# DUBSON0/iterative-closest-point-avmi

Measured on AMD Instinct MI355X. Metric: icp_iterations_per_sec, higher is better.
Workload: dtype f64

## Files before the change

### iterative-closest-point-avmi_amd/csrc/icp2.hip

```cpp
#include <cstdlib>

#include "linalg.hpp"
#include "prep_common.hpp"
#include "sweep.hpp"

namespace icpmi {


struct Icp2Args {
    const double* pts;
    const int32_t* off;
    const int32_t* cnt;
    const int32_t* pair_src;
    const int32_t* pair_tgt;
    const double* init;
    double* results;
    const double2* g_sxy;
    const double2* g_snrm;
    const int32_t* g_sorig;
    const float* g_skey;
    const int32_t* g_dir;
    int lds_points;
    double error_threshold;
    double max_corr_dist;
    int max_iterations;
    int method;
    int has_init;
    int n_lo, m_lo;
    int skip_over;
    int it_begin, it_limit;
    int resume;
    double2* st_xy;
    int32_t* st_pos;
    int32_t* list;
    int32_t* list_count;
    int st_stride;
    int32_t* wide_list;
    int32_t* wide_count;
    int32_t* far_list;
    int32_t* far_count;
    double far_d2;
    IcpGate gate;
};
constexpr int ICP2_FAR_THREADS = 1024, ICP2_FAR_SMAX = 2, ICP2_FAR_POINTS = 2048;
constexpr int ICP2_ST_PARKED = 100;

__device__ __forceinline__ double swap_add(double a, double b, bool rows16) {
    const long long ab = __double_as_longlong(a), bb = __double_as_longlong(b);
    const unsigned alo = (unsigned)ab, ahi = (unsigned)(ab >> 32), blo = (unsigned)bb, bhi = (unsigned)(bb >> 32);
    unsigned xl, xh, yl, yh;
    if (rows16) {
        const auto r0 = __builtin_amdgcn_permlane16_swap(alo, blo, false, false);
        const auto r1 = __builtin_amdgcn_permlane16_swap(ahi, bhi, false, false);
        xl = r0[0]; yl = r0[1]; xh = r1[0]; yh = r1[1];
    } else {
        const auto r0 = __builtin_amdgcn_permlane32_swap(alo, blo, false, false);
        const auto r1 = __builtin_amdgcn_permlane32_swap(ahi, bhi, false, false);
        xl = r0[0]; yl = r0[1]; xh = r1[0]; yh = r1[1];
    }
    return __longlong_as_double(((long long)xh << 32) | xl) + __longlong_as_double(((long long)yh << 32) | yl);
}

constexpr int RED_MAXW = 16;
template <int NV>
constexpr int red_doubles() { return (NV + 3) / 4 * 4 * RED_MAXW; }

template <int NV>
__device__ __forceinline__ void wave_totals(double* scratch, const double (&v)[NV]) {
    constexpr int NP = (NV + 3) / 4 * 4;
    const int w = wave_id(), l = lane_id();
    double h[NP / 2];
#pragma unroll
    for (int j = 0; j < NP / 2; ++j)
        h[j] = swap_add(2 * j < NV ? v[2 * j] : 0.0, 2 * j + 1 < NV ? v[2 * j + 1] : 0.0, false);
#pragma unroll
    for (int k = 0; k < NP / 4; ++k) {
        const double q = row_sum(swap_add(h[2 * k], h[2 * k + 1], true));
        const int row = l >> 4;
        const int idx = 4 * k + ((row & 1) << 1) + (row >> 1);
        if ((l & 15) == 0 && idx < NV) scratch[idx * RED_MAXW + w] = q;
    }
}

template <int NV>
__device__ __forceinline__ void combine_totals(const double* scratch, int n_waves, double (&v)[NV]) {
    const int l = lane_id();
    double s = 0.0;
    if (l < NV)
        for (int w = 0; w < n_waves; ++w) s += scratch[l * RED_MAXW + w];
#pragma unroll
    for (int i = 0; i < NV; ++i) v[i] = readlane_f64(s, i);
}

constexpr int CTRL_R = 0, CTRL_T = 4, CTRL_STOP = 6, CTRL_MP = 8, CTRL_MQ = 10;
constexpr int CTRL_RT = 12, CTRL_TT = 16, CTRL_ERR = 18, CTRL_PREV = 19, CTRL_DELTA = 20, CTRL_ITERS = 21, CTRL_STATUS = 22,
              CTRL_DOUBLES = 24;

#ifndef ICP2_STAGE1_ITERS
#define ICP2_STAGE1_ITERS 12
#endif
#ifndef ICP2_PK_MIN
#define ICP2_PK_MIN 16
#endif
#ifndef ICP2_PLAIN_ITERS
#define ICP2_PLAIN_ITERS 2
#endif
#ifndef ICP2_CENTRED_ITERS
#define ICP2_CENTRED_ITERS 2
#endif
#ifndef ICP2_PLAIN_CENTRED
#define ICP2_PLAIN_CENTRED ICP2_PLAIN_ITERS
#endif
__device__ __forceinline__ double wave_uniform(double v) {
    const long long b = __double_as_longlong(v);
    const unsigned lo = __builtin_amdgcn_readfirstlane((unsigned)b), hi = __builtin_amdgcn_readfirstlane((unsigned)(b >> 32));
    return __longlong_as_double((long long)(((unsigned long long)hi << 32) | lo));
}
__device__ __forceinline__ float wave_uniform(float v) {
    return __int_as_float(__builtin_amdgcn_readfirstlane(__float_as_int(v)));
}

constexpr int FIN_GO = 0, FIN_STOP = 1, FIN_FAR = 2;
__device__ __forceinline__ int finish_step(double* ctrl, int it, double err_sum, double inliers, int N, bool has_corr,
                                           int need, double error_threshold, bool writer, double far_err) {
    bool stop = false, far = false;
    if (it > 0) {
        const double err = err_sum / (double)N, delta = fabs(ctrl[CTRL_PREV] - err);
        stop = delta < error_threshold;
        far = it == 1 && err > far_err;
        if (writer) {
            ctrl[CTRL_ERR] = err; ctrl[CTRL_DELTA] = delta; ctrl[CTRL_PREV] = err; ctrl[CTRL_ITERS] = (double)it;
            if (stop) ctrl[CTRL_STATUS] = (double)ICPMI_ST_CONVERGED;
        }
    }
    if (!stop && has_corr && inliers < (double)need) {
        stop = true;
        if (writer) { ctrl[CTRL_STATUS] = (double)ICPMI_ST_FEW_INLIERS; ctrl[CTRL_ITERS] = (double)it; }
    }
    return stop ? FIN_STOP : (far ? FIN_FAR : FIN_GO);
}

__device__ __forceinline__ int gate_stop(double* ctrl, const int32_t* hint, int gate_seen, int gate_index, bool writer, int fin) {
    if (fin == FIN_STOP || !hint || __builtin_amdgcn_readfirstlane(gate_seen) >= gate_index) return fin;
    if (writer) ctrl[CTRL_STATUS] = (double)ICPMI_ST_SKIPPED;
    return FIN_STOP;
}

__device__ __forceinline__ void accumulate_step(double* ctrl, const double (&r)[4], const double (&t)[2]) {
    const double rt0 = ctrl[CTRL_RT], rt1 = ctrl[CTRL_RT + 1], rt2 = ctrl[CTRL_RT + 2], rt3 = ctrl[CTRL_RT + 3];
    const double tt0 = ctrl[CTRL_TT], tt1 = ctrl[CTRL_TT + 1];
    ctrl[CTRL_RT] = r[0] * rt0 + r[1] * rt2; ctrl[CTRL_RT + 1] = r[0] * rt1 + r[1] * rt3;
    ctrl[CTRL_RT + 2] = r[2] * rt0 + r[3] * rt2; ctrl[CTRL_RT + 3] = r[2] * rt1 + r[3] * rt3;
    ctrl[CTRL_TT] = (tt0 * r[0] + tt1 * r[1]) + t[0]; ctrl[CTRL_TT + 1] = (tt0 * r[2] + tt1 * r[3]) + t[1];
}

union FarSlot {
    struct { double x, y; int seed, pad; } in;
    struct { double s1, s3; int p1, p2; } out;
};
static_assert(sizeof(FarSlot) == 24, "24 B per row");

template <int THREADS, int ICP2_SMAX, bool TGT_LDS, bool FILT, bool RESUME, bool FAR = false>
__device__ __forceinline__ void icp2_pair(const Icp2Args& a, const int b) {
    extern __shared__ __attribute__((aligned(16))) unsigned char dyn[];
    __shared__ double redA[red_doubles<11>()];
    __shared__ double redB[red_doubles<4>()];
    __shared__ double ctrl[CTRL_DOUBLES];
    constexpr int NWAVES = THREADS / ICPMI_WAVE;

    const int tid = threadIdx.x;
    const bool lead = tid < ICPMI_WAVE;
    const int sc = a.pair_src[b], tc = a.pair_tgt[b];
    const int N = a.cnt ? a.cnt[sc] : a.off[sc + 1] - a.off[sc];
    const int M = a.cnt ? a.cnt[tc] : a.off[tc + 1] - a.off[tc];
    const double* src = a.pts + (size_t)a.off[sc] * 2;
    double* res = a.results + (size_t)b * ICPMI_RES_DOUBLES;
    const int dir = a.g_dir[tc];
    if (a.skip_over ? (N > THREADS * ICP2_SMAX || (TGT_LDS && M > a.lds_points)) : (a.n_lo >= 0 && N <= a.n_lo && M <= a.m_lo)) {
        if (a.skip_over && a.wide_list && threadIdx.x == 0) a.wide_list[atomicAdd(a.wide_count, 1)] = b;
        return;
    }
    const int gate_index = a.gate.base + b * a.gate.stride;
    if (RESUME && a.gate.hint) {
        __shared__ int gate_skip;
        if (tid == 0) {
            gate_skip = __hip_atomic_load(a.gate.hint, __ATOMIC_RELAXED, __HIP_MEMORY_SCOPE_AGENT) < gate_index;
            if (gate_skip) {
                res[ICPMI_RES_ITERS] += 1.0;
                res[ICPMI_RES_STATUS] = (double)ICPMI_ST_SKIPPED;
            }
        }
        __syncthreads();
        if (gate_skip) return;
    }
// ... 89 lines not shown
                    px[s] = sx; py[s] = sy;
                } else { px[s] = x; py[s] = y; }
            }
        }
        const bool has_corr = a.max_corr_dist >= 0.0;
        const double max_corr_sq = wave_uniform(a.max_corr_dist * a.max_corr_dist);
        const int need = max(3, N / 10);
        __syncthreads();
        if constexpr (FAR) {
            sweepf_build_tree(lds_sq, M, lds_tree, tree_leaves, tid, THREADS);
            __syncthreads();
        }
        const double2 c_lo = sxy[0], c_hi = sxy[M - 1];
        const double uabs = wave_uniform(fmax(fabs(proj(dir, c_lo.x, c_lo.y)), fabs(proj(dir, c_hi.x, c_hi.y))));
        if constexpr (FILT) {
            filt.rt = wave_uniform(__int_as_float(rt_bits) * 1.000001f);
            filt.ut = wave_uniform(fmaxf(fabsf(lds_sq[0].z), fabsf(lds_sq[M - 1].z)) * 1.000001f);
        }

        double e_part = 0.0;
        if (RESUME) {
#pragma unroll
            for (int s = 0; s < ICP2_SMAX; ++s) {
                if (!(s < S && s * THREADS + tid < N)) continue;
                const double2 q = sxy[pos[s]];
                const double ex = q.x - px[s], ey = q.y - py[s];
                double se = 0.0;
                se += ex * ex;
                se += ey * ey;
                e_part += se;
            }
        }
        bool stopped = false;
        const double far_err = !RESUME && a.max_iterations > 2 && N <= ICP2_FAR_THREADS * ICP2_FAR_SMAX && M <= ICP2_FAR_POINTS
                                   ? a.far_d2 : __builtin_inf();
        const int it_end = RESUME ? a.max_iterations : min(a.max_iterations, a.it_limit);
        for (int it = RESUME ? a.it_begin : 0; it < it_end; ++it) {
            int gate_seen = 0x7fffffff;
            if (a.gate.hint && tid == 0) gate_seen = __hip_atomic_load(a.gate.hint, __ATOMIC_RELAXED, __HIP_MEMORY_SCOPE_AGENT);
            bool srch[ICP2_SMAX];
#pragma unroll
            for (int s = 0; s < ICP2_SMAX; ++s) {
                const bool valid = s < S && s * THREADS + tid < N;
                bool within;
                if constexpr (FAR) {
                    within = false;
                    if (valid && budget[s] > 0.0f) {
                        const int pa = pos[s], pb = pos2[s] >= 0 ? pos2[s] : pos[s];
                        const double2 c = sxy[pa], e = sxy[pb];
                        const double dx = px[s] - c.x, dy = py[s] - c.y;
                        const double ex = px[s] - e.x, ey = py[s] - e.y;
                        double q2 = 0.0, w2 = 0.0;
                        q2 += dx * dx;
                        q2 += dy * dy;
                        w2 += ex * ex;
                        w2 += ey * ey;
                        const double g = (double)budget[s] - (fabs(px[s] - (double)ax[s]) + fabs(py[s] - (double)ay[s])) * 1.000000001;
                        within = g > 0.0 && fmin(q2, w2) * 1.000000000001 < g * g * 0.999999999999;
                    }
                } else {
                    within = valid && (fabs(px[s] - (double)ax[s]) + fabs(py[s] - (double)ay[s])) * 1.000000001 < (double)budget[s];
                }
                srch[s] = valid && !within;
                if (within) {
                    const int pa = pos[s], pb = pos2[s] >= 0 ? pos2[s] : pos[s];
                    const double2 c = sxy[pa], e = sxy[pb];
                    const double dx = px[s] - c.x, dy = py[s] - c.y;
                    const double ex = px[s] - e.x, ey = py[s] - e.y;
                    double q2 = 0.0, w2 = 0.0;
                    q2 += dx * dx;
                    q2 += dy * dy;
                    w2 += ex * ex;
                    w2 += ey * ey;
                    bool second_wins = w2 < q2;
                    if (w2 == q2 && pb != pa) {
                        if constexpr (FILT) second_wins = sweepf_row(lds_sq[pb]) < sweepf_row(lds_sq[pa]);
                        else second_wins = sorig[pb] < sorig[pa];
                    }
                    pos[s] = second_wins ? pb : pa;
                    pos2[s] = pos2[s] >= 0 ? (second_wins ? pa : pb) : -1;
                }
            }
            if (!RESUME && it < ICP2_PLAIN_ITERS) {
#pragma unroll
                for (int s = 0; s < ICP2_SMAX; ++s)
                    if (srch[s]) {
                        double d2s;
                        if constexpr (FILT) {
                            if (__popcll(__ballot(true)) >= ICP2_PK_MIN)
                                pos[s] = sweepf_nn_pk(lds_sq, sxy, filt, M, dir, uabs, px[s], py[s], pos[s], it < ICP2_PLAIN_CENTRED);
                            else pos[s] = sweepf_nn(lds_sq, sxy, filt, M, dir, uabs, px[s], py[s], pos[s], it < ICP2_PLAIN_CENTRED, d2s);
                        }
                        else pos[s] = sweep_nn(sxy, sorig, M, dir, uabs, px[s], py[s], pos[s], it < ICP2_PLAIN_CENTRED, d2s);
                    }
            } else {
                const bool centred = !RESUME && it < ICP2_CENTRED_ITERS;
                int slot[ICP2_SMAX];
                if constexpr (FAR) {
                    int nq = 0;
#pragma unroll
                    for (int s = 0; s < ICP2_SMAX; ++s) {
                        const unsigned long long bal = __ballot(srch[s]);
                        slot[s] = nq + (int)__builtin_amdgcn_mbcnt_hi((unsigned)(bal >> 32), __builtin_amdgcn_mbcnt_lo((unsigned)bal, 0u));
                        nq += __popcll(bal);
                        if (srch[s]) {
                            FarSlot e;
                            e.in.x = px[s]; e.in.y = py[s]; e.in.seed = pos[s]; e.in.pad = 0;
                            far_q[slot[s]] = e;
                        }
                    }
                    __builtin_amdgcn_fence(__ATOMIC_ACQ_REL, "wavefront");
                    __builtin_amdgcn_wave_barrier();
                    for (int j = tid & (ICPMI_WAVE - 1); j < nq; j += ICPMI_WAVE) {
                        const FarSlot e = far_q[j];
                        const Top2 r = sweepf_top2_far(lds_sq, sxy, lds_tree, tree_leaves, filt, M, dir, uabs, e.in.x, e.in.y, e.in.seed);
                        FarSlot o;
                        o.out.s1 = r.s1; o.out.s3 = r.s3; o.out.p1 = r.p1; o.out.p2 = r.p2;
                        far_q[j] = o;
                    }
                    __builtin_amdgcn_fence(__ATOMIC_ACQ_REL, "wavefront");
                    __builtin_amdgcn_wave_barrier();
                }
#pragma unroll
                for (int s = 0; s < ICP2_SMAX; ++s)
                    if (srch[s]) {
                        Top2 t2;
                        if constexpr (FAR) {
                            const FarSlot o = far_q[slot[s]];
                            t2.p1 = o.out.p1; t2.p2 = o.out.p2; t2.s1 = o.out.s1; t2.s2 = o.out.s1; t2.s3 = o.out.s3;
                        }
                        else if constexpr (FILT) {
                            if (__popcll(__ballot(true)) >= ICP2_PK_MIN)
                                t2 = sweepf_top2_pk(lds_sq, sxy, filt, M, dir, uabs, px[s], py[s], pos[s], centred);
                            else t2 = sweepf_top2(lds_sq, sxy, filt, M, dir, uabs, px[s], py[s], pos[s], centred);
                        }
                        else t2 = sweep_top2(sxy, sorig, M, dir, uabs, px[s], py[s], pos[s], centred);
                        pos[s] = t2.p1; pos2[s] = t2.p2;
                        float bf;
                        if constexpr (FAR) {
                            const double d1 = sqrt(t2.s1), d3 = sqrt(t2.s3);
                            bf = (float)(d3 - 1e-13 * (d3 + d1) - 1.3e-7 * (fabs(px[s]) + fabs(py[s])));
                        } else {
                            const float r3 = __builtin_amdgcn_sqrtf((float)t2.s3) * 0.9999997f;
                            const float r1 = __builtin_amdgcn_sqrtf((float)t2.s1) * 1.0000003f + 1e-30f;
                            bf = (r3 - r1) * 0.4999999f - 1.3e-7f * (fabsf((float)px[s]) + fabsf((float)py[s]));
                        }
                        bf = bf - fabsf(bf) * 1e-6f;
                        budget[s] = t2.s3 < __builtin_inf() ? bf : __builtin_inff();
                        ax[s] = (float)px[s]; ay[s] = (float)py[s];
                    }
            }
            bool in[ICP2_SMAX];
#pragma unroll
            for (int s = 0; s < ICP2_SMAX; ++s) in[s] = s < S && s * THREADS + tid < N;
            if (use_p2l) {
                double acc[11] = {0, 0, 0, 0, 0, 0, 0, 0, 0, 0, 0};
#pragma unroll
                for (int s = 0; s < ICP2_SMAX; ++s) {
                    if (!in[s]) continue;
                    const double2 q = sxy[pos[s]], nm = snrm[pos[s]];
                    const double dx = px[s] - q.x, dy = py[s] - q.y;
                    if (has_corr) {
                        double s2 = 0.0;
                        s2 += dx * dx;
                        s2 += dy * dy;
                        const double dist = sqrt(s2);
                        if (!(dist * dist < max_corr_sq)) continue;
                    }
                    const double c = nm.y * px[s] - nm.x * py[s];
                    const double bi = -(nm.x * dx + nm.y * dy);
                    acc[0] += c * c;       acc[1] += c * nm.x;    acc[2] += c * nm.y;
                    acc[3] += nm.x * nm.x; acc[4] += nm.x * nm.y; acc[5] += nm.y * nm.y;
                    acc[6] += c * bi;      acc[7] += nm.x * bi;   acc[8] += nm.y * bi;
                    acc[9] += 1.0;
                }
                acc[10] = e_part;
                wave_totals<11>(redA, acc);
                __syncthreads();
                if (lead) {
                    combine_totals<11>(redA, NWAVES, acc);
                    const int fin = gate_stop(ctrl, a.gate.hint, gate_seen, gate_index, tid == 0,
                                              finish_step(ctrl, it, acc[10], acc[9], N, has_corr, need, a.error_threshold, tid == 0, far_err));
                    const bool stop = fin == FIN_STOP;
                    if (!stop) {
                        double A[3][3] = {{acc[0], acc[1], acc[2]}, {acc[1], acc[3], acc[4]}, {acc[2], acc[4], acc[5]}};
                        double rhs[3] = {acc[6], acc[7], acc[8]}, x[3];
                        double r[4], t[2];
                        if (solve3(A, rhs, x)) {
                            double st, ct;
                            sincos_step(x[0], st, ct);
                            r[0] = ct; r[1] = -st; r[2] = st; r[3] = ct; t[0] = x[1]; t[1] = x[2];
                        } else {
                            r[0] = 1.0; r[1] = 0.0; r[2] = 0.0; r[3] = 1.0; t[0] = 0.0; t[1] = 0.0;
                        }
                        if (tid == 0) {
                            accumulate_step(ctrl, r, t);
                            ctrl[CTRL_R] = r[0]; ctrl[CTRL_R + 1] = r[1]; ctrl[CTRL_R + 2] = r[2]; ctrl[CTRL_R + 3] = r[3];
                            ctrl[CTRL_T] = t[0]; ctrl[CTRL_T + 1] = t[1];
                        }
                    }
                    if (tid == 0) ctrl[CTRL_STOP] = (double)fin;
                }
                __syncthreads();
            } else {
                double m[6] = {0, 0, 0, 0, 0, 0};
#pragma unroll
                for (int s = 0; s < ICP2_SMAX; ++s) {
                    if (!in[s]) continue;
                    const double2 q = sxy[pos[s]];
                    if (has_corr) {
                        const double dx = px[s] - q.x, dy = py[s] - q.y;
                        double s2 = 0.0;
                        s2 += dx * dx;
                        s2 += dy * dy;
                        const double dist = sqrt(s2);
                        in[s] = dist * dist < max_corr_sq;
                        if (!in[s]) continue;
                    }
                    m[0] += px[s]; m[1] += py[s]; m[2] += q.x; m[3] += q.y; m[4] += 1.0;
                }
                m[5] = e_part;
                wave_totals<6>(redA, m);
                __syncthreads();
                if (lead) {
                    combine_totals<6>(redA, NWAVES, m);
                    const int fin = gate_stop(ctrl, a.gate.hint, gate_seen, gate_index, tid == 0,
                                              finish_step(ctrl, it, m[5], m[4], N, has_corr, need, a.error_threshold, tid == 0, far_err));
                    if (tid == 0) {
                        ctrl[CTRL_STOP] = (double)fin;
                        ctrl[CTRL_MP] = m[0] / m[4]; ctrl[CTRL_MP + 1] = m[1] / m[4];
                        ctrl[CTRL_MQ] = m[2] / m[4]; ctrl[CTRL_MQ + 1] = m[3] / m[4];
                    }
                }
// ... 172 lines not shown
    if (points > 1024 && points <= 1536) cap = 1536;
    const bool filter = in_lds && cap <= 2048;
    const size_t lds = in_lds ? (filter ? (size_t)cap * 48 + 32 : (size_t)cap * 36) : 0;
    return {threads, smax, in_lds, filter, cap, lds, -1, 0, 0};
}

static Icp2Plan plan_icp2(int n_pairs, int max_src_n, int max_tgt_n, const icpmi_icp_params& p, bool have_ws,
                          const char* stages_opt, const char* far_opt) {
    Icp2Plan plan{};
    const bool in_lds = max_tgt_n <= 4096;
    const bool many = n_pairs >= 1024;
    int T, SM;
    if (max_src_n <= 1024) { T = 512; SM = 2; }
    else if (many) { T = 768; SM = 2; }
    else if (max_src_n <= 2048) { T = 1024; SM = 2; }
    else { T = 1024; SM = 4; }
    const int cap1 = ((T == 512 || T == 768) && many && in_lds && max_tgt_n > 1536) ? 1536 : max_tgt_n;
    plan.first = icp2_shape(T, SM, cap1, in_lds);
    plan.has_wide = T * SM < max_src_n || cap1 < max_tgt_n;
    if (plan.has_wide) {
        plan.first.skip_over = 1;
        plan.wide = icp2_shape(1024, max_src_n <= 2048 ? 2 : 4, max_tgt_n, in_lds);
        plan.wide.n_lo = T * SM; plan.wide.m_lo = cap1;
    }
    plan.stage1_iterations = ICP2_STAGE1_ITERS;
    plan.two_stage = many && have_ws && p.max_iterations >= 2 * plan.stage1_iterations &&
                     !(stages_opt && stages_opt[0] == '1') &&
                     (p.method == ICPMI_POINT_TO_LINE || (stages_opt && stages_opt[0] == '2'));
    plan.stage2_grid = n_pairs / 8 > 256 ? n_pairs / 8 : 256;
    plan.wide_grid = n_pairs < 256 ? n_pairs : (n_pairs / 32 > 256 ? n_pairs / 32 : 256);
    plan.far_d2 = far_opt ? atof(far_opt) : 1.0;
    plan.far_wanted = have_ws && in_lds && plan.far_d2 > 0.0 && p.max_iterations > 2;
    int far_cap = 64;
    while (far_cap < max_tgt_n && far_cap < ICP2_FAR_POINTS) far_cap <<= 1;
    plan.far = {ICP2_FAR_THREADS, ICP2_FAR_SMAX, true, true, far_cap,
                (size_t)far_cap * 50 + 32 + sizeof(FarSlot) * (size_t)(ICP2_FAR_THREADS * ICP2_FAR_SMAX), -1, 0, 0};
    plan.needs_lists = have_ws && (plan.two_stage || plan.has_wide);
    return plan;
}

struct Icp2Kernels {
    void (*fused)(Icp2Args);
    void (*wide)(Icp2Args);
    void (*resume)(Icp2Args);
    void (*resume_rest)(Icp2Args, int);
};
template <int T, int S, bool L, bool F>
constexpr Icp2Kernels icp2_kernels() {
    return {icp2_fused_kernel<T, S, L, F>, icp2_wide_kernel<T, S, L, F>, icp2_resume_kernel<T, S, L, F>,
            icp2_resume_rest_kernel<T, S, L, F>};
}
template <int T, int S>
static Icp2Kernels icp2_kernels_of(const Icp2Shape& s) {
    if (!s.in_lds) return icp2_kernels<T, S, false, false>();
    if (s.filter) return icp2_kernels<T, S, true, true>();
    return icp2_kernels<T, S, true, false>();
}
static Icp2Kernels icp2_kernels_of(const Icp2Shape& s) {
    if (s.threads == 512 && s.smax == 2) return icp2_kernels_of<512, 2>(s);
    if (s.threads == 768 && s.smax == 2) return icp2_kernels_of<768, 2>(s);
    if (s.threads == 1024 && s.smax == 2) return icp2_kernels_of<1024, 2>(s);
    if (s.threads == 1024 && s.smax == 4) return icp2_kernels_of<1024, 4>(s);
    return {nullptr, nullptr, nullptr, nullptr};
}

static Icp2Args icp2_args(const Icp2Args& base, const Icp2Shape& s, int it_begin, int it_limit, int resume) {
    Icp2Args a = base;
    a.lds_points = s.lds_points; a.n_lo = s.n_lo; a.m_lo = s.m_lo; a.skip_over = s.skip_over;
    a.it_begin = it_begin; a.it_limit = it_limit; a.resume = resume;
    return a;
}

int launch_icp2(const double* pts, const int32_t* off, const int32_t* cnt, const int32_t* ps, const int32_t* pt,
                int n_pairs, int max_src_n, int max_tgt_n, int total_rows, const icpmi_icp_params* p, const double* init,
                double* results, const void* prepared, void* workspace, size_t workspace_bytes, const IcpGate* gate,
                hipStream_t st) {
    const Icp2Ws w{workspace, n_pairs, max_src_n};
    const bool have_ws = workspace && workspace_bytes >= w.bytes;
    const Icp2Plan plan = plan_icp2(n_pairs, max_src_n, max_tgt_n, *p, have_ws, option("ICP2_STAGES"), option("ICP2_FAR"));
    const Icp2Kernels k1 = icp2_kernels_of(plan.first), k2 = icp2_kernels_of(plan.wide);
    if (!k1.fused || (plan.has_wide && !k2.fused)) return ICPMI_ERR_ARG;
    Icp2Args base;
    base.gate = gate ? *gate : IcpGate{nullptr, nullptr, 0.0, 0, 1};
    base.st_xy = nullptr; base.st_pos = nullptr; base.list = nullptr; base.list_count = nullptr; base.st_stride = 0;
    base.wide_list = nullptr; base.wide_count = nullptr;
    base.far_list = nullptr; base.far_count = nullptr; base.far_d2 = __builtin_inf();
    const PreparedView v(prepared, total_rows);
    base.pts = pts; base.off = off; base.cnt = cnt; base.pair_src = ps; base.pair_tgt = pt; base.init = init; base.results = results;
    base.g_sxy = v.sxy; base.g_snrm = v.snrm; base.g_sorig = v.sorig; base.g_skey = v.skey; base.g_dir = v.dir;
    base.error_threshold = p->error_threshold; base.max_corr_dist = p->max_corr_dist;
    base.max_iterations = p->max_iterations; base.method = p->method; base.has_init = p->has_init;
    const bool far_go = plan.far_wanted && dyn_lds((const void*)icp2_far_kernel, plan.far.lds) == hipSuccess;
    if (plan.needs_lists || far_go) {
        base.st_xy = w.st_xy; base.st_pos = w.st_pos; base.st_stride = max_src_n;
        base.list = w.list; base.list_count = w.list_count;
        if (plan.has_wide) { base.wide_list = w.wide_list; base.wide_count = w.list_count + 1; }
        if (far_go) { base.far_list = w.far_list; base.far_count = w.list_count + 2; base.far_d2 = plan.far_d2; }
        if (hipMemsetAsync(w.list_count, 0, 3 * sizeof(int32_t), st) != hipSuccess) return ICPMI_ERR_HIP;
    }
    SideLock side_lock;
    Side* const side = side_lock.side;

    const Icp2Shape& s1 = plan.first;
    if (dyn_lds((const void*)k1.fused, s1.lds) != hipSuccess) return ICPMI_ERR_HIP;
    k1.fused<<<n_pairs, s1.threads, s1.lds, st>>>(
        icp2_args(base, s1, 0, plan.two_stage ? plan.stage1_iterations : ICP2_NO_LIMIT, 0));
    bool forked = false;
    if (plan.two_stage) {
        if (base.wide_list && side) forked = hipEventRecord(side->fork, st) == hipSuccess;
        const Icp2Args second = icp2_args(base, s1, plan.stage1_iterations, ICP2_NO_LIMIT, 1);
        if (dyn_lds((const void*)k1.resume, s1.lds) != hipSuccess) return ICPMI_ERR_HIP;
        k1.resume<<<plan.stage2_grid, s1.threads, s1.lds, st>>>(second);
        if (plan.stage2_grid < n_pairs) {
            if (dyn_lds((const void*)k1.resume_rest, s1.lds) != hipSuccess) return ICPMI_ERR_HIP;
            k1.resume_rest<<<256, s1.threads, s1.lds, st>>>(second, plan.stage2_grid);
        }
    }
    if (plan.has_wide) {
        const Icp2Shape& s2 = plan.wide;
        const Icp2Args wide = icp2_args(base, s2, 0, ICP2_NO_LIMIT, 0);
        if (base.wide_list) {
            if (dyn_lds((const void*)k2.wide, s2.lds) != hipSuccess) return ICPMI_ERR_HIP;
            hipStream_t ws = st;
            if (forked && hipStreamWaitEvent(side->stream[0], side->fork, 0) == hipSuccess) ws = side->stream[0];
            k2.wide<<<plan.wide_grid, s2.threads, s2.lds, ws>>>(wide);
            if (ws != st && (hipEventRecord(side->join[0], ws) != hipSuccess ||
                             hipStreamWaitEvent(st, side->join[0], 0) != hipSuccess)) {
                (void)hipStreamSynchronize(ws);
                return ICPMI_ERR_HIP;
            }
        } else {
            if (dyn_lds((const void*)k2.fused, s2.lds) != hipSuccess) return ICPMI_ERR_HIP;
            k2.fused<<<n_pairs, s2.threads, s2.lds, st>>>(wide);
        }
    }
    if (base.far_list)
        icp2_far_kernel<<<n_pairs < 256 ? n_pairs : 256, plan.far.threads, plan.far.lds, st>>>(
            icp2_args(base, plan.far, 2, ICP2_NO_LIMIT, 1));
    ICPMI_LAUNCH_CHECK();
    return ICPMI_OK;
}

}
```

### iterative-closest-point-avmi_amd/csrc/state.hip

```cpp
#include <link.h>

#include <cstdio>
#include <cstdlib>
#include <cstring>
#include <map>
#include <set>
#include <mutex>
#include <string>

#include "common.hpp"

namespace icpmi {

static const char* const kOptionNames[] = {"ICP2_SIDE", "ICP2_FAR", "ICP2_STAGES", "POLAR", "PREP_KNN", "RAYCAST", "RS_BATCH"};

struct Options {
    std::mutex mu;
    bool loaded = false;
    std::map<std::string, std::string> values;
    void load() {
        if (loaded) return;
        loaded = true;
        for (const char* n : kOptionNames) {
            const std::string env = std::string("ICPMI_") + n;
            if (const char* v = getenv(env.c_str())) values[n] = v;
        }
    }
};
static Options& options() { static Options o; return o; }

static const char* strip_prefix(const char* name) { return strncmp(name, "ICPMI_", 6) == 0 ? name + 6 : name; }

const char* option(const char* name) {
    Options& o = options();
    std::lock_guard<std::mutex> g(o.mu);
    o.load();
    const auto it = o.values.find(strip_prefix(name));
    return it == o.values.end() ? nullptr : it->second.c_str();
}

struct LdsAttr {
    std::mutex mu;
    std::map<std::pair<const void*, int>, size_t> granted;
};
static LdsAttr& lds_attr() { static LdsAttr a; return a; }

hipError_t dyn_lds(const void* fn, size_t bytes) {
    int dev = -1;
    hipError_t e = hipGetDevice(&dev);
    if (e != hipSuccess) return e;
    LdsAttr& a = lds_attr();
    std::lock_guard<std::mutex> g(a.mu);
    size_t& have = a.granted[std::make_pair(fn, dev)];
    if (bytes <= have) return hipSuccess;
    e = hipFuncSetAttribute(fn, hipFuncAttributeMaxDynamicSharedMemorySize, (int)bytes);
    if (e == hipSuccess) have = bytes;
    return e;
}

struct SideState {
    std::mutex mu;
    std::map<int, Side> per_device;
};
static SideState& side_state() { static SideState s; return s; }

SideLock::SideLock() : side(nullptr) {
    SideState& s = side_state();
    s.mu.lock();
    const char* e = option("ICP2_SIDE");
    if (e && e[0] == '0') return;
    int dev = -1;
    if (hipGetDevice(&dev) != hipSuccess) return;
    Side& sd = s.per_device[dev];
    if (sd.failed) return;
    if (!sd.fork) {
        bool ok = hipEventCreateWithFlags(&sd.fork, hipEventDisableTiming) == hipSuccess;
        for (int i = 0; ok && i < ICPMI_SIDE_STREAMS; ++i)
            ok = hipStreamCreateWithFlags(&sd.stream[i], hipStreamNonBlocking) == hipSuccess &&
                 hipEventCreateWithFlags(&sd.join[i], hipEventDisableTiming) == hipSuccess;
        if (!ok) { sd.failed = true; return; }
    }
    side = &sd;
}
SideLock::~SideLock() { side_state().mu.unlock(); }

}

extern "C" int icpmi_set_option(const char* name, const char* value) {
    using namespace icpmi;
    if (!name) return ICPMI_ERR_ARG;
    const char* n = strip_prefix(name);
    bool known = false;
    for (const char* k : kOptionNames) known = known || strcmp(k, n) == 0;
    if (!known) return ICPMI_ERR_ARG;
    Options& o = options();
    std::lock_guard<std::mutex> g(o.mu);
    o.load();
// ... 44 lines not shown
```

### iterative-closest-point-avmi_amd/csrc/sweep.hpp

```cpp
#pragma once
#include "common.hpp"

namespace icpmi {

__device__ __forceinline__ double proj(int dir, double x, double y) {
    const double a = dir == 1 ? 0.0 : 1.0;
    const double b = dir == 0 ? 0.0 : (dir == 3 ? -1.0 : 1.0);
    return x * a + y * b;
}

__device__ __forceinline__ bool gap_exceeds(int dir, double uq, double uc, double bound_d2) {
    const double du = fabs(uq - uc);
    if (dir < 2) return du * du > bound_d2;
    const double e = 4.5e-16 * (fabs(uq) + fabs(uc));
    const double l = du - e;
    return l > 0.0 && l * l > bound_d2 * 2.000000000000002;
}

__device__ __forceinline__ int sweep_lower_bound(const double2* sxy, int m, int dir, double uq) {
    int lo = 0, hi = m;
    while (lo < hi) {
        const int mid = (lo + hi) >> 1;
        const double2 c = sxy[mid];
        if (proj(dir, c.x, c.y) < uq) lo = mid + 1; else hi = mid;
// ... 447 lines not shown
        L.offer(sweep_pk(s2.x, hp, inr && hp != skip));
        L.offer(sweep_pk(s2.y, lp, inl && lp != skip));
        if (!(inr || inl)) return true;
        if (max_rounds > 0 && ++rounds >= max_rounds) return false;
        W = fq.width<POLAR>(fq.dist_bound(L.m[NB]));
        hi += inr ? 1 : 0;
        lo -= inl ? 1 : 0;
    }
}

template <int K, int NB>
__device__ __forceinline__ void sweep_pk_search(const float4* sq, const SweepPkQuery& fq, int m, int seed, bool CENTRED, SweepPkList<K>& L) {
    const bool seeded = seed >= 0 && seed < m;
    int skip = -1;
    const bool from_seed = seeded && !CENTRED && !(fq.polar && fabsf(sq[seed].z - fq.u) > 3.0f);
    if (seeded && !from_seed) {
        const float4 c = sq[seed];
        const float ex = fq.x - c.x, ey = fq.y - c.y;
        L.offer(sweep_pk(__builtin_fmaf(ex, ex, ey * ey), seed, true));
        skip = seed;
    }
    const int h0 = from_seed ? seed + 1 : sweepf_lower_bound(sq, m, fq.u);
    if (fq.polar) sweep_pk_walk<K, NB, true>(sq, fq, h0 - 1, h0, m, skip, L);
    else sweep_pk_walk<K, NB, false>(sq, fq, h0 - 1, h0, m, skip, L);
}

__device__ __forceinline__ int sweepf_nn_pk(const float4* sq, const double2* sxy, const SweepF& f, int m, int dir, double uabs,
                                            double qx, double qy, int seed, bool CENTRED) {
    const SweepPkQuery fq(f, dir, uabs, qx, qy);
    SweepPkList<3> L;
    sweep_pk_search<3, 0>(sq, fq, m, seed, CENTRED, L);
    const float T = fq.threshold(fq.dist_bound(L.m[0]));
    int bpos = (int)(L.m[0] & SWEEP_PK_IDX);
    const bool a2 = L.m[1] != SWEEP_PK_NONE && !(sweep_pk_floor(L.m[1]) > T);
    const bool a3 = L.m[2] != SWEEP_PK_NONE && !(sweep_pk_floor(L.m[2]) > T);
    if (a3 || fq.bad || L.m[0] == SWEEP_PK_NONE) {
        double d2;
        bpos = sweepf_nn(sq, sxy, f, m, dir, uabs, qx, qy, seed, CENTRED, d2);
    } else if (a2) {
        const int i2 = (int)(L.m[1] & SWEEP_PK_IDX);
        const double s1 = sweep_d2(qx, qy, sxy[bpos]), s2 = sweep_d2(qx, qy, sxy[i2]);
        if (s2 < s1 || (s2 == s1 && sweepf_row(sq[i2]) < sweepf_row(sq[bpos]))) bpos = i2;
    }
    return bpos;
}

__device__ __forceinline__ Top2 sweep_pk_top2_exact(const float4* sq, const double2* sxy, double qx, double qy, unsigned w0, unsigned w1, unsigned w2) {
    const unsigned w[3] = {w0, w1, w2};
    double s[3];
    int p[3], r[3];
#pragma unroll
    for (int k = 0; k < 3; ++k) {
        const bool have = w[k] != SWEEP_PK_NONE;
        p[k] = have ? (int)(w[k] & SWEEP_PK_IDX) : -1;
        const int j = have ? p[k] : 0;
        s[k] = have ? sweep_d2(qx, qy, sxy[j]) : __builtin_inf();
        r[k] = have ? sweepf_row(sq[j]) : 0x7fffffff;
    }
#define ICPMI_CS(a, b)                                                                              \
    do {                                                                                            \
        const bool sw = s[b] < s[a] || (s[b] == s[a] && r[b] < r[a]);                              \
        const double sa = sw ? s[b] : s[a], sb = sw ? s[a] : s[b];                                  \
        const int pa = sw ? p[b] : p[a], pb = sw ? p[a] : p[b], ra = sw ? r[b] : r[a], rb = sw ? r[a] : r[b]; \
        s[a] = sa; s[b] = sb; p[a] = pa; p[b] = pb; r[a] = ra; r[b] = rb;                           \
    } while (0)
    ICPMI_CS(0, 1); ICPMI_CS(1, 2); ICPMI_CS(0, 1);
#undef ICPMI_CS
    Top2 t;
    t.p1 = p[0]; t.p2 = p[1]; t.s1 = s[0]; t.s2 = s[1]; t.s3 = s[2];
    return t;
}

__device__ __forceinline__ Top2 sweepf_top2_pk(const float4* sq, const double2* sxy, const SweepF& f, int m, int dir, double uabs,
                                               double qx, double qy, int seed, bool CENTRED) {
    const SweepPkQuery fq(f, dir, uabs, qx, qy);
    SweepPkList<4> L;
    sweep_pk_search<4, 2>(sq, fq, m, seed, CENTRED, L);
    const float T = fq.threshold(fq.dist_bound(L.m[2]));
    const bool a4 = L.m[3] != SWEEP_PK_NONE && !(sweep_pk_floor(L.m[3]) > T);
    if (a4 || fq.bad || L.m[0] == SWEEP_PK_NONE) return sweepf_top2(sq, sxy, f, m, dir, uabs, qx, qy, seed, CENTRED);
    return sweep_pk_top2_exact(sq, sxy, qx, qy, L.m[0], L.m[1], L.m[2]);
}

constexpr int SWEEP_BLOCK = 16;
#ifndef SWEEP_FAR_ROUNDS
#define SWEEP_FAR_ROUNDS 24
#endif

__host__ __device__ __forceinline__ int sweepf_tree_leaves(int m) {
    int l = 2;
    while (l * SWEEP_BLOCK < m) l <<= 1;
    return l;
}

__device__ __forceinline__ void sweepf_build_tree(const float4* sq, int m, float4* tree, int leaves, int tid, int nthreads) {
    for (int b = tid; b < leaves; b += nthreads) {
        const int i1 = min(m, (b + 1) * SWEEP_BLOCK);
        float x0 = __builtin_inff(), y0 = __builtin_inff(), x1 = -__builtin_inff(), y1 = -__builtin_inff();
        for (int i = b * SWEEP_BLOCK; i < i1; ++i) {
            const float4 c = sq[i];
            x0 = fminf(x0, c.x); y0 = fminf(y0, c.y); x1 = fmaxf(x1, c.x); y1 = fmaxf(y1, c.y);
        }
        tree[leaves + b] = make_float4(x0, y0, x1, y1);
    }
    __syncthreads();
    for (int k = 1 + tid; k < leaves; k += nthreads) {
        int lo = k, hi = k;
        while (lo < leaves) { lo = 2 * lo; hi = 2 * hi + 1; }
        float x0 = __builtin_inff(), y0 = __builtin_inff(), x1 = -__builtin_inff(), y1 = -__builtin_inff();
        for (int j = lo; j <= hi; ++j) {
            const float4 c = tree[j];
            x0 = fminf(x0, c.x); y0 = fminf(y0, c.y); x1 = fmaxf(x1, c.z); y1 = fmaxf(y1, c.w);
        }
        tree[k] = make_float4(x0, y0, x1, y1);
    }
}

__device__ __forceinline__ float sweepf_box_s2(const float4 bb, float qx, float qy) {
    const float dx = fmaxf(fmaxf(bb.x - qx, qx - bb.z), 0.0f), dy = fmaxf(fmaxf(bb.y - qy, qy - bb.w), 0.0f);
    return __builtin_fmaf(dx, dx, dy * dy);
}

template <class Offer>
__device__ __forceinline__ void sweepf_far_scan(const float4* sq, const float4* tree, int leaves, int m, const SweepFQuery& fq,
                                                const float& T, Offer offer) {
    int node = 1;
    unsigned trail = 0;
    bool tested = true;
    for (;;) {
        bool down = tested || !(sweepf_box_s2(tree[node], fq.x, fq.y) > T);
        if (down && node < leaves) {
            const float la = sweepf_box_s2(tree[2 * node], fq.x, fq.y), lb = sweepf_box_s2(tree[2 * node + 1], fq.x, fq.y);
            const bool b_first = lb < la;
            const float l_near = b_first ? lb : la, l_far = b_first ? la : lb;
            if (!(l_near > T)) {
                trail = (trail << 1) | (l_far > T ? 0u : 1u);
                node = 2 * node + (b_first ? 1 : 0);
                tested = true;
                continue;
            }
            down = false;
        }
        if (down) {
            const int b = node - leaves;
#pragma unroll
            for (int e = 0; e < SWEEP_BLOCK / 8; ++e) {
                const int i0 = b * SWEEP_BLOCK + e * 8;
                float v[8];
#pragma unroll
                for (int k = 0; k < 8; ++k) {
                    const float2 c = *reinterpret_cast<const float2*>(sq + i0 + k);
                    const float ex = fq.x - c.x, ey = fq.y - c.y;
                    v[k] = __builtin_fmaf(ex, ex, ey * ey);
                }
#pragma unroll
                for (int k = 0; k < 8; ++k)
                    if (!(v[k] > T) && i0 + k < m) offer(i0 + k);
            }
        }
        if (trail == 0) break;
        const int up = __builtin_ctz(trail);
        node = (node >> up) ^ 1;
        trail = (trail >> up) ^ 1u;
        tested = false;
    }
}
// ... 190 lines not shown
```

Baseline: 42.08 million.

## Compact two sparse search slots into one wave pass via lane permutes

When both per-thread search slots have active lanes and their combined count fits in a wavefront, the queries are packed into contiguous lanes with ds_permute. A single top-2 sweep then runs for both slots instead of two divergent serial passes, and the results are pulled back with ds_bpermute. This targets lane underuse from divergence in the correspondence search. It adds permute traffic, packs p1 and p2 into 16 bits each (this assumes indices fit in 16 bits), and adds a diagnostic census compiled only under ICPMI_DIAG. The packed path is on by default and can be disabled through the ICP2_PACK option.

```diff
diff --git a/iterative-closest-point-avmi_amd/csrc/icp2.hip b/iterative-closest-point-avmi_amd/csrc/icp2.hip
--- a/iterative-closest-point-avmi_amd/csrc/icp2.hip
+++ b/iterative-closest-point-avmi_amd/csrc/icp2.hip
@@ -1,3 +1,4 @@
+#include <cstdio>
 #include <cstdlib>
 
 #include "linalg.hpp"
@@ -41,6 +42,7 @@
     int32_t* far_count;
     double far_d2;
     IcpGate gate;
+    int pack;
 };
 constexpr int ICP2_FAR_THREADS = 1024, ICP2_FAR_SMAX = 2, ICP2_FAR_POINTS = 2048;
 constexpr int ICP2_ST_PARKED = 100;
@@ -110,6 +112,26 @@
 #endif
 #ifndef ICP2_PLAIN_CENTRED
 #define ICP2_PLAIN_CENTRED ICP2_PLAIN_ITERS
+#endif
+#ifdef ICPMI_DIAG
+constexpr int CENSUS_ITERS = 16, CENSUS_COLS = 10;
+__device__ unsigned long long icp2_census[CENSUS_ITERS][CENSUS_COLS];
+__device__ __forceinline__ void icp2_census_add(int it, int n0, int n1) {
+    if ((threadIdx.x & (ICPMI_WAVE - 1)) == 0) {
+        unsigned long long* c = icp2_census[it < CENSUS_ITERS ? it : CENSUS_ITERS - 1];
+        const bool both = n0 > 0 && n1 > 0, fits = both && n0 + n1 <= ICPMI_WAVE;
+        const unsigned long long v[CENSUS_COLS] = {
+            1ull, (unsigned long long)(n0 + n1 > 0), (unsigned long long)(n0 + n1), (unsigned long long)((n0 > 0) + (n1 > 0)),
+            (unsigned long long)both, (unsigned long long)fits, (unsigned long long)((n0 >= ICP2_PK_MIN) + (n1 >= ICP2_PK_MIN)),
+            (unsigned long long)(fits && n0 + n1 >= ICP2_PK_MIN),
+            (unsigned long long)(fits ? (n0 >= ICP2_PK_MIN) + (n1 >= ICP2_PK_MIN) : 0), (unsigned long long)(fits ? n0 + n1 : 0)};
+        for (int k = 0; k < CENSUS_COLS; ++k)
+            if (v[k]) atomicAdd(&c[k], v[k]);
+    }
+}
+#define ICP2_CENSUS(it, n0, n1) icp2_census_add(it, n0, n1)
+#else
+#define ICP2_CENSUS(it, n0, n1) ((void)0)
 #endif
 __device__ __forceinline__ double wave_uniform(double v) {
     const long long b = __double_as_longlong(v);
@@ -365,6 +387,7 @@
                 }
             }
             if (!RESUME && it < ICP2_PLAIN_ITERS) {
+                if constexpr (FILT && ICP2_SMAX == 2) ICP2_CENSUS(it, (int)__popcll(__ballot(srch[0])), (int)__popcll(__ballot(srch[1])));
 #pragma unroll
                 for (int s = 0; s < ICP2_SMAX; ++s)
                     if (srch[s]) {
@@ -404,34 +427,61 @@
                     __builtin_amdgcn_fence(__ATOMIC_ACQ_REL, "wavefront");
                     __builtin_amdgcn_wave_barrier();
                 }
-#pragma unroll
-                for (int s = 0; s < ICP2_SMAX; ++s)
-                    if (srch[s]) {
+                auto keep = [&](int s, const Top2& t2) {
+                    pos[s] = t2.p1; pos2[s] = t2.p2;
+                    float bf;
+                    if constexpr (FAR) {
+                        const double d1 = sqrt(t2.s1), d3 = sqrt(t2.s3);
+                        bf = (float)(d3 - 1e-13 * (d3 + d1) - 1.3e-7 * (fabs(px[s]) + fabs(py[s])));
+                    } else {
+                        const float r3 = __builtin_amdgcn_sqrtf((float)t2.s3) * 0.9999997f;
+                        const float r1 = __builtin_amdgcn_sqrtf((float)t2.s1) * 1.0000003f + 1e-30f;
+                        bf = (r3 - r1) * 0.4999999f - 1.3e-7f * (fabsf((float)px[s]) + fabsf((float)py[s]));
+                    }
+                    bf = bf - fabsf(bf) * 1e-6f;
+                    budget[s] = t2.s3 < __builtin_inf() ? bf : __builtin_inff();
+                    ax[s] = (float)px[s]; ay[s] = (float)py[s];
+                };
+                bool packed = false;
+                if constexpr (FILT && !FAR && ICP2_SMAX == 2 && !(RESUME && THREADS == 768)) {
+                    const SweepSlotPack sp(srch[0], srch[1]);
+                    ICP2_CENSUS(it, sp.n0, sp.n1);
+                    if (a.pack && sp.applies()) {
+                        packed = true;
+                        double qx, qy;
+                        int seed;
+                        sp.gather(srch[0], srch[1], px, py, pos, qx, qy, seed);
                         Top2 t2;
-                        if constexpr (FAR) {
-                            const FarSlot o = far_q[slot[s]];
-                            t2.p1 = o.out.p1; t2.p2 = o.out.p2; t2.s1 = o.out.s1; t2.s2 = o.out.s1; t2.s3 = o.out.s3;
+                        t2.p1 = 0; t2.p2 = -1; t2.s1 = t2.s2 = t2.s3 = 0.0;
+                        if ((tid & (ICPMI_WAVE - 1)) < sp.rows()) {
+                            if (sp.rows() >= ICP2_PK_MIN) t2 = sweepf_top2_pk(lds_sq, sxy, filt, M, dir, uabs, qx, qy, seed, centred);
+                            else t2 = sweepf_top2(lds_sq, sxy, filt, M, dir, uabs, qx, qy, seed, centred);
                         }
-                        else if constexpr (FILT) {
-                            if (__popcll(__ballot(true)) >= ICP2_PK_MIN)
-                                t2 = sweepf_top2_pk(lds_sq, sxy, filt, M, dir, uabs, px[s], py[s], pos[s], centred);
-                            else t2 = sweepf_top2(lds_sq, sxy, filt, M, dir, uabs, px[s], py[s], pos[s], centred);
+#pragma unroll
+                        for (int s = 0; s < ICP2_SMAX; ++s) {
+                            const Top2 r = sp.answer(s, t2);
+                            if (srch[s]) keep(s, r);
                         }
-                        else t2 = sweep_top2(sxy, sorig, M, dir, uabs, px[s], py[s], pos[s], centred);
-                        pos[s] = t2.p1; pos2[s] = t2.p2;
-                        float bf;
-                        if constexpr (FAR) {
-                            const double d1 = sqrt(t2.s1), d3 = sqrt(t2.s3);
-                            bf = (float)(d3 - 1e-13 * (d3 + d1) - 1.3e-7 * (fabs(px[s]) + fabs(py[s])));
-                        } else {
-                            const float r3 = __builtin_amdgcn_sqrtf((float)t2.s3) * 0.9999997f;
-                            const float r1 = __builtin_amdgcn_sqrtf((float)t2.s1) * 1.0000003f + 1e-30f;
-                            bf = (r3 - r1) * 0.4999999f - 1.3e-7f * (fabsf((float)px[s]) + fabsf((float)py[s]));
+                    }
+                }
+                if (!packed) {
+#pragma unroll
+                    for (int s = 0; s < ICP2_SMAX; ++s)
+                        if (srch[s]) {
+                            Top2 t2;
+                            if constexpr (FAR) {
+                                const FarSlot o = far_q[slot[s]];
+                                t2.p1 = o.out.p1; t2.p2 = o.out.p2; t2.s1 = o.out.s1; t2.s2 = o.out.s1; t2.s3 = o.out.s3;
+                            }
+                            else if constexpr (FILT) {
+                                if (__popcll(__ballot(true)) >= ICP2_PK_MIN)
+                                    t2 = sweepf_top2_pk(lds_sq, sxy, filt, M, dir, uabs, px[s], py[s], pos[s], centred);
+                                else t2 = sweepf_top2(lds_sq, sxy, filt, M, dir, uabs, px[s], py[s], pos[s], centred);
+                            }
+                            else t2 = sweep_top2(sxy, sorig, M, dir, uabs, px[s], py[s], pos[s], centred);
+                            keep(s, t2);
                         }
-                        bf = bf - fabsf(bf) * 1e-6f;
-                        budget[s] = t2.s3 < __builtin_inf() ? bf : __builtin_inff();
-                        ax[s] = (float)px[s]; ay[s] = (float)py[s];
-                    }
+                }
             }
             bool in[ICP2_SMAX];
 #pragma unroll
@@ -770,6 +820,8 @@
     if (!k1.fused || (plan.has_wide && !k2.fused)) return ICPMI_ERR_ARG;
     Icp2Args base;
     base.gate = gate ? *gate : IcpGate{nullptr, nullptr, 0.0, 0, 1};
+    const char* pack_opt = option("ICP2_PACK");
+    base.pack = !(pack_opt && pack_opt[0] == '0');
     base.st_xy = nullptr; base.st_pos = nullptr; base.list = nullptr; base.list_count = nullptr; base.st_stride = 0;
     base.wide_list = nullptr; base.wide_count = nullptr;
     base.far_list = nullptr; base.far_count = nullptr; base.far_d2 = __builtin_inf();
@@ -826,6 +878,21 @@
         icp2_far_kernel<<<n_pairs < 256 ? n_pairs : 256, plan.far.threads, plan.far.lds, st>>>(
             icp2_args(base, plan.far, 2, ICP2_NO_LIMIT, 1));
     ICPMI_LAUNCH_CHECK();
+#ifdef ICPMI_DIAG
+    if (option("ICP2_CENSUS")) {
+        static unsigned long long c[CENSUS_ITERS][CENSUS_COLS];
+        if (hipStreamSynchronize(st) != hipSuccess || hipMemcpyFromSymbol(c, HIP_SYMBOL(icp2_census), sizeof(c)) != hipSuccess) return ICPMI_ERR_HIP;
+        fprintf(stderr, "icp2 census (%d pairs): it waves searching rows walks both both<=64 pk_walks fit_pk(n0+n1>=%d) fit_pk_walks fit_rows\n", n_pairs, ICP2_PK_MIN);
+        for (int i = 0; i < CENSUS_ITERS; ++i) {
+            if (!c[i][0]) continue;
+            fprintf(stderr, "icp2 census %2d", i);
+            for (int k = 0; k < CENSUS_COLS; ++k) fprintf(stderr, " %llu", c[i][k]);
+            fprintf(stderr, "\n");
+        }
+        static const unsigned long long zero[CENSUS_ITERS][CENSUS_COLS] = {};
+        if (hipMemcpyToSymbol(HIP_SYMBOL(icp2_census), zero, sizeof(zero)) != hipSuccess) return ICPMI_ERR_HIP;
+    }
+#endif
     return ICPMI_OK;
 }
 
diff --git a/iterative-closest-point-avmi_amd/csrc/state.hip b/iterative-closest-point-avmi_amd/csrc/state.hip
--- a/iterative-closest-point-avmi_amd/csrc/state.hip
+++ b/iterative-closest-point-avmi_amd/csrc/state.hip
@@ -12,7 +12,7 @@
 
 namespace icpmi {
 
-static const char* const kOptionNames[] = {"ICP2_SIDE", "ICP2_FAR", "ICP2_STAGES", "POLAR", "PREP_KNN", "RAYCAST", "RS_BATCH"};
+static const char* const kOptionNames[] = {"ICP2_SIDE", "ICP2_FAR", "ICP2_STAGES", "ICP2_PACK", "ICP2_CENSUS", "POLAR", "PREP_KNN", "RAYCAST", "RS_BATCH"};
 
 struct Options {
     std::mutex mu;
diff --git a/iterative-closest-point-avmi_amd/csrc/sweep.hpp b/iterative-closest-point-avmi_amd/csrc/sweep.hpp
--- a/iterative-closest-point-avmi_amd/csrc/sweep.hpp
+++ b/iterative-closest-point-avmi_amd/csrc/sweep.hpp
@@ -553,6 +553,56 @@
     return sweep_pk_top2_exact(sq, sxy, qx, qy, L.m[0], L.m[1], L.m[2]);
 }
 
+__device__ __forceinline__ int sweep_lanes_below(unsigned long long bal) {
+    return (int)__builtin_amdgcn_mbcnt_hi((unsigned)(bal >> 32), __builtin_amdgcn_mbcnt_lo((unsigned)bal, 0u));
+}
+__device__ __forceinline__ double sweep_push_f64(int to, double v) {
+    const long long b = __double_as_longlong(v);
+    const unsigned lo = (unsigned)__builtin_amdgcn_ds_permute(to << 2, (int)(unsigned)b);
+    const unsigned hi = (unsigned)__builtin_amdgcn_ds_permute(to << 2, (int)(unsigned)(b >> 32));
+    return __longlong_as_double((long long)(((unsigned long long)hi << 32) | lo));
+}
+__device__ __forceinline__ double sweep_pull_f64(int from, double v) {
+    const long long b = __double_as_longlong(v);
+    const unsigned lo = (unsigned)__builtin_amdgcn_ds_bpermute(from << 2, (int)(unsigned)b);
+    const unsigned hi = (unsigned)__builtin_amdgcn_ds_bpermute(from << 2, (int)(unsigned)(b >> 32));
+    return __longlong_as_double((long long)(((unsigned long long)hi << 32) | lo));
+}
+struct SweepSlotPack {
+    unsigned long long bal0, bal1;
+    int n0, n1;
+    __device__ __forceinline__ SweepSlotPack(bool s0, bool s1) {
+        bal0 = __ballot(s0); bal1 = __ballot(s1);
+        n0 = __popcll(bal0); n1 = __popcll(bal1);
+    }
+    __device__ __forceinline__ bool applies() const { return n0 > 0 && n1 > 0 && n0 + n1 <= 64; }
+    __device__ __forceinline__ int rows() const { return n0 + n1; }
+    __device__ __forceinline__ int runner(int slot) const {
+        return slot == 0 ? sweep_lanes_below(bal0) : (n0 + sweep_lanes_below(bal1)) & 63;
+    }
+    __device__ __forceinline__ void gather(bool s0, bool s1, const double (&px)[2], const double (&py)[2], const int (&pos)[2],
+                                           double& qx, double& qy, int& seed) const {
+        const int lane = sweep_lanes_below(~0ull);
+        const int idle0 = lane - sweep_lanes_below(bal0), idle1 = lane - sweep_lanes_below(bal1);
+        const int to0 = s0 ? runner(0) : n0 + idle0;
+        const int to1 = s1 ? runner(1) : (idle1 < n0 ? idle1 : idle1 + n1);
+        const double x0 = sweep_push_f64(to0, px[0]), y0 = sweep_push_f64(to0, py[0]);
+        const int p0 = __builtin_amdgcn_ds_permute(to0 << 2, pos[0]);
+        const double x1 = sweep_push_f64(to1, px[1]), y1 = sweep_push_f64(to1, py[1]);
+        const int p1 = __builtin_amdgcn_ds_permute(to1 << 2, pos[1]);
+        const bool first = lane < n0;
+        qx = first ? x0 : x1; qy = first ? y0 : y1; seed = first ? p0 : p1;
+    }
+    __device__ __forceinline__ Top2 answer(int slot, const Top2& t) const {
+        const int from = runner(slot);
+        const int pp = __builtin_amdgcn_ds_bpermute(from << 2, (int)(((unsigned)t.p1 & 0xffffu) | ((unsigned)t.p2 << 16)));
+        Top2 r;
+        r.p1 = pp & 0xffff; r.p2 = pp >> 16;
+        r.s1 = sweep_pull_f64(from, t.s1); r.s2 = r.s1; r.s3 = sweep_pull_f64(from, t.s3);
+        return r;
+    }
+};
+
 constexpr int SWEEP_BLOCK = 16;
 #ifndef SWEEP_FAR_ROUNDS
 #define SWEEP_FAR_ROUNDS 24
```

Result: no change. 41.89 million (-0.5%).
